# zhoujoey/ORB-SLAM3-Mac

Measured on AMD Instinct MI355X. Metric: ORB extract+match frames/sec, higher is better.
Workload: dtype u8; 1 GPU; vga: synthetic 640x480 batch=1024 per GPU, 8-level pyramid, 1000 feats/frame, ORB extract + Hamming 2-NN match (Frame.cc:1146) + SearchForInitialization (ORBmatcher.cc:710) vs successor frame; pipelines=1, matchers=side by side (two contexts), frames_total=1024

## Files before the change

orb-slam3-mac_amd/csrc/bf2nn_kernels.hip:

```cpp
#include "orb_internal.h"
#include "ctx_internal.h"
#include <climits>
#include <cstdlib>
#include <cstring>
#include <type_traits>

extern "C" int orbhip_descriptor_distance(const uint8_t *a32, const uint8_t *b32)
{
    int dist = 0;
    for (int i = 0; i < 8; i++) {
        uint32_t pa, pb;
        memcpy(&pa, a32 + 4 * i, 4); memcpy(&pb, b32 + 4 * i, 4);
        uint32_t v = pa ^ pb;
        v = v - ((v >> 1) & 0x55555555);
        v = (v & 0x33333333) + ((v >> 2) & 0x33333333);
        dist += (((v + (v >> 4)) & 0xF0F0F0F) * 0x1010101) >> 24;
    }
    return dist;
}

#define BF_TILE 256
__device__ __forceinline__ bool bf_slice(const int32_t *nA, const int32_t *nB, const int32_t *monoA, const int32_t *monoB, int pair, int max_n,
                                         int &na, int &nb, int &ma, int &mb)
{
    na = nA[pair]; nb = nB[pair]; ma = 0; mb = 0;
    if (!monoA) return true;
    if (na > max_n || nb > max_n) return false;
    ma = min(max(monoA[pair], 0), max(na, 0)); mb = min(max(monoB[pair], 0), max(nb, 0));
    na -= ma; nb -= mb;
    return true;
}
template <bool MONO>
__global__ __launch_bounds__(256) void k_bf2nn(const uint8_t *descA, const int32_t *nA, size_t strideA,
                                               const uint8_t *descB, const int32_t *nB, size_t strideB,
                                               int max_n, double ratio, int32_t *idx2, int32_t *dist2, uint8_t *accept,
                                               const int32_t *monoA, const int32_t *monoB)
{
    __shared__ uint4 tile[BF_TILE * 2];
    const int pair = blockIdx.y, tid = threadIdx.x;
    int na, nb, ma, mb;
    if (!bf_slice(nA, nB, MONO ? monoA : nullptr, monoB, pair, max_n, na, nb, ma, mb)) return;
    const int q = blockIdx.x * 256 + tid;
    if (blockIdx.x * 256 >= na) return;
    const uint4 *A = reinterpret_cast<const uint4 *>(descA + (size_t)pair * strideA) + 2 * (size_t)ma;
    const uint4 *B = reinterpret_cast<const uint4 *>(descB + (size_t)pair * strideB) + 2 * (size_t)mb;
    uint4 a0 = make_uint4(0, 0, 0, 0), a1 = a0;
    if (q < na) { a0 = A[2 * q]; a1 = A[2 * q + 1]; }
    uint32_t kb = 0xFFFFFFFFu, ks = 0xFFFFFFFFu;
    for (int t0 = 0; t0 < nb; t0 += BF_TILE) {
        const int tn = min(BF_TILE, nb - t0);
        __syncthreads();
        for (int i = tid; i < tn * 2; i += 256) tile[i] = B[2 * t0 + i];
        __syncthreads();
#pragma unroll 4
        for (int j = 0; j < tn; j++) {
            const uint32_t key = ((uint32_t)hamming256(a0, a1, tile[2 * j], tile[2 * j + 1]) << 16) | (uint32_t)(t0 + j);
            ks = min(ks, max(kb, key));
            kb = min(kb, key);
        }
    }
    if (q < na) {
        const int best = kb == 0xFFFFFFFFu ? INT_MAX : (int)(kb >> 16), second = ks == 0xFFFFFFFFu ? INT_MAX : (int)(ks >> 16);
        const int bi = kb == 0xFFFFFFFFu ? -1 : (int)(kb & 0xFFFFu), si = ks == 0xFFFFFFFFu ? -1 : (int)(ks & 0xFFFFu);
        const size_t o = ((size_t)pair * max_n + q) * 2;
        idx2[o] = bi; idx2[o + 1] = si; dist2[o] = best; dist2[o + 1] = second;
        accept[(size_t)pair * max_n + q] = (si >= 0 && (double)(float)best < (double)(float)second * ratio) ? 1 : 0;
    }
}

#define BFM_ROWB 272
typedef int bfm_v4i __attribute__((ext_vector_type(4)));
typedef int bfm_v16i __attribute__((ext_vector_type(16)));
__device__ __forceinline__ uint32_t bfm_widen4(uint32_t nib) { return __umul24(nib, 0x00204081u) & 0x01010101u; }
__device__ __forceinline__ uint32_t bfm_widen4_pm(uint32_t nib)
{
    const uint32_t s = bfm_widen4(nib);
    return ((s << 8) - s) | 0x01010101u;
}
#define BFM_WAVES 8
template <bool MONO>
__global__ __launch_bounds__(64 * BFM_WAVES, 4) void k_bf2nn_mfma(const uint8_t *descA, const int32_t *nA, size_t strideA,
                                                    const uint8_t *descB, const int32_t *nB, size_t strideB,
                                                    int max_n, double ratio, int32_t *idx2, int32_t *dist2, uint8_t *accept,
                                                    const int32_t *monoA, const int32_t *monoB)
{
    __shared__ __attribute__((aligned(16))) uint8_t Bx[2 * 64 * BFM_ROWB];
    static_assert(BFM_WAVES * 2 * 8 * 64 * 4 <= 2 * 64 * BFM_ROWB, "the merge area (half of the rows at a time) fits the tile buffers");
    const int pair = blockIdx.y, tid = threadIdx.x, lane = tid & 63, wave = tid >> 6;
    int na, nb, ma, mb;
    if (!bf_slice(nA, nB, MONO ? monoA : nullptr, monoB, pair, max_n, na, nb, ma, mb)) return;
    const int q0 = blockIdx.x * (32 * BFM_WAVES);
    if (q0 >= na) return;
    const uint32_t *A = reinterpret_cast<const uint32_t *>(descA + (size_t)pair * strideA) + 8 * (size_t)ma;
    const uint32_t *B = reinterpret_cast<const uint32_t *>(descB + (size_t)pair * strideB) + 8 * (size_t)mb;
    const int r = lane & 31, h = lane >> 5;
    const int qrow = q0 + 32 * wave + r;
    bfm_v4i af[8];
    int pa_row = 0;
    {
        uint32_t w[8];
#pragma unroll
        for (int m = 0; m < 8; m++) { w[m] = qrow < na ? A[(size_t)8 * qrow + m] : 0u; pa_row += __popc(w[m]); }
#pragma unroll
        for (int m = 0; m < 8; m++) {
            const uint32_t hw = (w[m] >> (16 * h)) & 0xFFFFu;
            af[m] = (bfm_v4i){(int)bfm_widen4_pm(hw & 15u), (int)bfm_widen4_pm((hw >> 4) & 15u), (int)bfm_widen4_pm((hw >> 8) & 15u), (int)bfm_widen4_pm(hw >> 12)};
        }
        asm volatile("" : "+v"(pa_row));
    }
    uint32_t k1[16], k2[16];
#pragma unroll
    for (int g = 0; g < 16; g++) { k1[g] = 0xFFFFFFFFu; k2[g] = 0xFFFFFFFFu; }
    const int sc = tid >> 3, sm = tid & 7;
    auto fetch = [&](int t0, uint32_t &w0) { w0 = (t0 + sc < nb) ? B[(uint32_t)(8 * (t0 + sc) + sm)] : 0u; };
    auto widen = [&](int bufi, uint32_t w) {
        uint4 lo = make_uint4(bfm_widen4(w & 15u), bfm_widen4((w >> 4) & 15u), bfm_widen4((w >> 8) & 15u), bfm_widen4((w >> 12) & 15u));
        uint4 hi = make_uint4(bfm_widen4((w >> 16) & 15u), bfm_widen4((w >> 20) & 15u), bfm_widen4((w >> 24) & 15u), bfm_widen4(w >> 28));
        uint4 *dst = reinterpret_cast<uint4 *>(&Bx[bufi * 64 * BFM_ROWB + sc * BFM_ROWB + sm * 32]);
        dst[0] = lo; dst[1] = hi;
    };
    uint32_t nw0;
    fetch(0, nw0);
    widen(0, nw0);
    __syncthreads();
    const bfm_v16i zero = {0, 0, 0, 0, 0, 0, 0, 0, 0, 0, 0, 0, 0, 0, 0, 0};
    bfm_v16i accA = zero, accB = zero;
    uint32_t baseB = 0;
    auto retire = [&](const bfm_v16i &acc, uint32_t base, int g) {
        const uint32_t key = ((uint32_t)acc[g] << 16) + base;
        asm("v_med3_u32 %1, %0, %2, %1\n\tv_min_u32 %0, %0, %2" : "+v"(k1[g]), "+v"(k2[g]) : "v"(key));
    };
    auto key_base = [&](int col) { return (col < nb ? (uint32_t)col : (0x40000000u | (uint32_t)col)) + (256u << 16); };
    const uint8_t *bx0 = &Bx[r * BFM_ROWB + h * 16];
    int buf = 0, t0 = 0;
    auto tile = [&](auto first) {
        constexpr bool FIRST = decltype(first)::value;
        const bool more = t0 + 64 < nb;
        if (more) fetch(t0 + 64, nw0);
        const uint8_t *bx = bx0 + buf * 64 * BFM_ROWB;
        auto rd = [&](int q) { return *reinterpret_cast<const bfm_v4i *>(bx + (q >> 3) * 32 * BFM_ROWB + (q & 7) * 32); };
        bfm_v4i bq[4];
#pragma unroll
        for (int q = 0; q < 4; q++) bq[q] = rd(q);
        if constexpr (!FIRST) {
#pragma unroll
            for (int g = 0; g < 4; g++) retire(accB, baseB, g);
        }
        const uint32_t baseA = key_base(t0 + r);
#pragma unroll
        for (int m = 0; m < 8; m++) {
            accA = __builtin_amdgcn_mfma_i32_32x32x32_i8(af[m], bq[m & 3], m ? accA : zero, 0, 0, 0);
            bq[m & 3] = rd(m + 4);
            if constexpr (!FIRST) {
                retire(accB, baseB, 4 + 3 * (m >> 1) + 2 * (m & 1));
                if (!(m & 1)) retire(accB, baseB, 5 + 3 * (m >> 1));
            }
            __builtin_amdgcn_sched_barrier(0);
        }
        baseB = key_base(t0 + 32 + r);
#pragma unroll
        for (int m = 0; m < 8; m++) {
            accB = __builtin_amdgcn_mfma_i32_32x32x32_i8(af[m], bq[m & 3], m ? accB : zero, 0, 0, 0);
            if (m < 4) bq[m & 3] = rd(m + 12);
            if (m) {
                const int g0 = (16 * (m - 1) + 6) / 7, g1 = (16 * m + 6) / 7;
#pragma unroll
                for (int g = g0; g < g1; g++) retire(accA, baseA, g);
            }
            __builtin_amdgcn_sched_barrier(0);
        }
        if (more) widen(buf ^ 1, nw0);
        __syncthreads();
        t0 += 64; buf ^= 1;
    };
    if (32 < nb) tile(std::true_type());
    while (t0 + 32 < nb) tile(std::false_type());
    if (t0 < nb) {
        const uint8_t *bx = bx0 + buf * 64 * BFM_ROWB;
        bfm_v4i bq[8];
#pragma unroll
        for (int m = 0; m < 8; m++) bq[m] = *reinterpret_cast<const bfm_v4i *>(bx + m * 32);
#pragma unroll
        for (int m = 0; m < 8; m++) accA = __builtin_amdgcn_mfma_i32_32x32x32_i8(af[m], bq[m], m ? accA : zero, 0, 0, 0);
        if (t0) {
#pragma unroll
            for (int g = 0; g < 16; g++) retire(accB, baseB, g);
        }
        const uint32_t baseA = key_base(t0 + r);
#pragma unroll
        for (int g = 0; g < 16; g++) retire(accA, baseA, g);
        __syncthreads();
    } else if (nb > 0) {
#pragma unroll
        for (int g = 0; g < 16; g++) retire(accB, baseB, g);
    }
    uint32_t (*kout)[2][8][64] = reinterpret_cast<uint32_t (*)[2][8][64]>(&Bx[0]);
#pragma unroll
    for (int part = 0; part < 2; part++) {
        if (part) __syncthreads();
#pragma unroll
        for (int g = 0; g < 8; g++) { kout[wave][0][g][lane] = k1[8 * part + g]; kout[wave][1][g][lane] = k2[8 * part + g]; }
        __syncthreads();
        const int row = 16 * part + (lane >> 2), g = (row & 3) + 4 * ((row >> 3) & 1), hh = (row >> 2) & 1;
        const int unbias = __shfl(pa_row, row, 64) - 256;
        uint32_t kb = 0xFFFFFFFFu, ks = 0xFFFFFFFFu;
#pragma unroll
        for (int c = 0; c < 8; c++) {
            const int cc = 32 * hh + 8 * (lane & 3) + ((c + (lane >> 2)) & 7);
            const uint32_t a1 = kout[wave][0][g][cc], a2 = kout[wave][1][g][cc];
            ks = min(min(ks, a2), max(kb, a1));
            kb = min(kb, a1);
        }
#pragma unroll
        for (int s = 1; s < 4; s <<= 1) {
            const uint32_t pb = __shfl_xor(kb, s, 64), ps = __shfl_xor(ks, s, 64);
            ks = min(min(ks, ps), max(kb, pb));
            kb = min(kb, pb);
        }
        const int q = q0 + 32 * wave + row;
        if ((lane & 3) == 0 && q < na) {
            const bool hb = !(kb & 0x40000000u), hs = !(ks & 0x40000000u);
            const int best = hb ? (int)(kb >> 16) + unbias : INT_MAX, second = hs ? (int)(ks >> 16) + unbias : INT_MAX;
            const int bi = hb ? (int)(kb & 0xFFFFu) : -1, si = hs ? (int)(ks & 0xFFFFu) : -1;
            const size_t o = ((size_t)pair * max_n + q) * 2;
            idx2[o] = bi; idx2[o + 1] = si; dist2[o] = best; dist2[o + 1] = second;
            accept[(size_t)pair * max_n + q] = (si >= 0 && (double)(float)best < (double)(float)second * ratio) ? 1 : 0;
        }
    }
}

extern "C" int orbhip_match_bf2nn_device(orbhip_ctx *ctx, const uint8_t *d_descA, const int32_t *d_nA, size_t strideA,
                                         const uint8_t *d_descB, const int32_t *d_nB, size_t strideB, int pairs,
                                         int max_n, double ratio, int32_t *d_idx2, int32_t *d_dist2, uint8_t *d_accept)
{
    if (!ctx || !d_descA || !d_descB || !d_nA || !d_nB || pairs <= 0 || max_n <= 0 || max_n > 65535 || !d_idx2 || !d_dist2 || !d_accept)
        return ORBHIP_E_BADARG;
    if (hipSetDevice(orbhip_ctx_device_internal(ctx)) != hipSuccess) return ORBHIP_E_HIP;
    if (max_n >= 64 && !getenv("ORBHIP_BF2NN_VALU")) {
        dim3 grid((max_n + 32 * BFM_WAVES - 1) / (32 * BFM_WAVES), pairs);
        hipLaunchKernelGGL(k_bf2nn_mfma<false>, grid, dim3(64 * BFM_WAVES), 0, orbhip_ctx_stream_internal(ctx), d_descA, d_nA, strideA, d_descB, d_nB,
                           strideB, max_n, ratio, d_idx2, d_dist2, d_accept, nullptr, nullptr);
    } else {
        dim3 grid((max_n + 255) / 256, pairs);
        hipLaunchKernelGGL(k_bf2nn<false>, grid, dim3(256), 0, orbhip_ctx_stream_internal(ctx), d_descA, d_nA, strideA, d_descB, d_nB,
                           strideB, max_n, ratio, d_idx2, d_dist2, d_accept, nullptr, nullptr);
    }
    return hipGetLastError() == hipSuccess ? ORBHIP_OK : ORBHIP_E_HIP;
}

int orbhip_bf2nn_slices_internal(orbhip_ctx *ctx, const uint8_t *d_descA, const int32_t *d_nA, const int32_t *d_monoA, size_t strideA,
                                 const uint8_t *d_descB, const int32_t *d_nB, const int32_t *d_monoB, size_t strideB, int pairs, int max_n,
                                 double ratio, int32_t *d_idx2, int32_t *d_dist2, uint8_t *d_accept)
{
    if (max_n >= 64 && !getenv("ORBHIP_BF2NN_VALU")) {
        dim3 grid((max_n + 32 * BFM_WAVES - 1) / (32 * BFM_WAVES), pairs);
        hipLaunchKernelGGL(k_bf2nn_mfma<true>, grid, dim3(64 * BFM_WAVES), 0, orbhip_ctx_stream_internal(ctx), d_descA, d_nA, strideA, d_descB, d_nB,
                           strideB, max_n, ratio, d_idx2, d_dist2, d_accept, d_monoA, d_monoB);
    } else {
        dim3 grid((max_n + 255) / 256, pairs);
        hipLaunchKernelGGL(k_bf2nn<true>, grid, dim3(256), 0, orbhip_ctx_stream_internal(ctx), d_descA, d_nA, strideA, d_descB, d_nB,
                           strideB, max_n, ratio, d_idx2, d_dist2, d_accept, d_monoA, d_monoB);
    }
    return hipGetLastError() == hipSuccess ? ORBHIP_OK : ORBHIP_E_HIP;
}
```

Measured before the change: 363,500 frames/s.

## Fold column index into MFMA accumulator to skip per-element key building

```diff
diff --git a/orb-slam3-mac_amd/csrc/bf2nn_kernels.hip b/orb-slam3-mac_amd/csrc/bf2nn_kernels.hip
--- a/orb-slam3-mac_amd/csrc/bf2nn_kernels.hip
+++ b/orb-slam3-mac_amd/csrc/bf2nn_kernels.hip
@@ -78,7 +78,15 @@
     return ((s << 8) - s) | 0x01010101u;
 }
 #define BFM_WAVES 8
-template <bool MONO>
+#define BFM_S 64
+#define BFM_NONE 0xFC000
+__device__ __forceinline__ uint32_t bfm_widen4_pmS(uint32_t nib)
+{
+    uint32_t s = bfm_widen4(nib);
+    asm("" : "+v"(s));
+    return (s << 7) | 0x40404040u;
+}
+template <bool MONO, bool TIDX>
 __global__ __launch_bounds__(64 * BFM_WAVES, 4) void k_bf2nn_mfma(const uint8_t *descA, const int32_t *nA, size_t strideA,
                                                     const uint8_t *descB, const int32_t *nB, size_t strideB,
                                                     int max_n, double ratio, int32_t *idx2, int32_t *dist2, uint8_t *accept,
@@ -91,6 +99,7 @@
     if (!bf_slice(nA, nB, MONO ? monoA : nullptr, monoB, pair, max_n, na, nb, ma, mb)) return;
     const int q0 = blockIdx.x * (32 * BFM_WAVES);
     if (q0 >= na) return;
+    if (TIDX && nb > 32 * BFM_S) return;
     const uint32_t *A = reinterpret_cast<const uint32_t *>(descA + (size_t)pair * strideA) + 8 * (size_t)ma;
     const uint32_t *B = reinterpret_cast<const uint32_t *>(descB + (size_t)pair * strideB) + 8 * (size_t)mb;
     const int r = lane & 31, h = lane >> 5;
@@ -104,13 +113,14 @@
 #pragma unroll
         for (int m = 0; m < 8; m++) {
             const uint32_t hw = (w[m] >> (16 * h)) & 0xFFFFu;
-            af[m] = (bfm_v4i){(int)bfm_widen4_pm(hw & 15u), (int)bfm_widen4_pm((hw >> 4) & 15u), (int)bfm_widen4_pm((hw >> 8) & 15u), (int)bfm_widen4_pm(hw >> 12)};
+            if constexpr (TIDX) af[m] = (bfm_v4i){(int)bfm_widen4_pmS(hw & 15u), (int)bfm_widen4_pmS((hw >> 4) & 15u), (int)bfm_widen4_pmS((hw >> 8) & 15u), (int)bfm_widen4_pmS(hw >> 12)};
+            else af[m] = (bfm_v4i){(int)bfm_widen4_pm(hw & 15u), (int)bfm_widen4_pm((hw >> 4) & 15u), (int)bfm_widen4_pm((hw >> 8) & 15u), (int)bfm_widen4_pm(hw >> 12)};
         }
         asm volatile("" : "+v"(pa_row));
     }
     uint32_t k1[16], k2[16];
 #pragma unroll
-    for (int g = 0; g < 16; g++) { k1[g] = 0xFFFFFFFFu; k2[g] = 0xFFFFFFFFu; }
+    for (int g = 0; g < 16; g++) { k1[g] = TIDX ? (uint32_t)BFM_NONE : 0xFFFFFFFFu; k2[g] = k1[g]; }
     const int sc = tid >> 3, sm = tid & 7;
     auto fetch = [&](int t0, uint32_t &w0) { w0 = (t0 + sc < nb) ? B[(uint32_t)(8 * (t0 + sc) + sm)] : 0u; };
     auto widen = [&](int bufi, uint32_t w) {
@@ -127,21 +137,49 @@
     bfm_v16i accA = zero, accB = zero;
     uint32_t baseB = 0;
     auto retire = [&](const bfm_v16i &acc, uint32_t base, int g) {
-        const uint32_t key = ((uint32_t)acc[g] << 16) + base;
-        asm("v_med3_u32 %1, %0, %2, %1\n\tv_min_u32 %0, %0, %2" : "+v"(k1[g]), "+v"(k2[g]) : "v"(key));
+        if constexpr (TIDX) {
+            if (g == 0) {
+                const int x = acc[0], b1 = (int)k1[0], b2 = (int)k2[0];
+                k2[0] = (uint32_t)max(min(b2, x), min(max(b2, x), b1));
+                k1[0] = (uint32_t)min(b1, x);
+                asm volatile("" : "+v"(k1[0]), "+v"(k2[0]));
+            } else {
+                asm volatile("v_med3_i32 %1, %0, %2, %1\n\tv_min_i32 %0, %0, %2" : "+v"(k1[g]), "+v"(k2[g]) : "v"(acc[g]));
+            }
+        } else {
+            const uint32_t key = ((uint32_t)acc[g] << 16) + base;
+            asm("v_med3_u32 %1, %0, %2, %1\n\tv_min_u32 %0, %0, %2" : "+v"(k1[g]), "+v"(k2[g]) : "v"(key));
+        }
     };
+    auto retire_last = [&](const bfm_v16i &acc, int col0, uint32_t base) {
+        if constexpr (TIDX) {
+            const bool real = col0 + r < nb;
+#pragma unroll
+            for (int g = 0; g < 16; g++) {
+                const int x = real ? acc[g] : BFM_NONE;
+                asm volatile("v_med3_i32 %1, %0, %2, %1\n\tv_min_i32 %0, %0, %2" : "+v"(k1[g]), "+v"(k2[g]) : "v"(x));
+            }
+        } else {
+#pragma unroll
+            for (int g = 0; g < 16; g++) retire(acc, base, g);
+        }
+    };
+    const long a9 = h ? 0 : 1;
+    auto open_chain = [&](int col0) { return __builtin_amdgcn_mfma_i32_32x32x16_i8(a9, (long)(col0 >> 5), zero, 0, 0, 0); };
     auto key_base = [&](int col) { return (col < nb ? (uint32_t)col : (0x40000000u | (uint32_t)col)) + (256u << 16); };
     const uint8_t *bx0 = &Bx[r * BFM_ROWB + h * 16];
     int buf = 0, t0 = 0;
+    constexpr int RING = TIDX ? 2 : 4;
     auto tile = [&](auto first) {
         constexpr bool FIRST = decltype(first)::value;
         const bool more = t0 + 64 < nb;
         if (more) fetch(t0 + 64, nw0);
         const uint8_t *bx = bx0 + buf * 64 * BFM_ROWB;
         auto rd = [&](int q) { return *reinterpret_cast<const bfm_v4i *>(bx + (q >> 3) * 32 * BFM_ROWB + (q & 7) * 32); };
-        bfm_v4i bq[4];
-#pragma unroll
-        for (int q = 0; q < 4; q++) bq[q] = rd(q);
+        bfm_v4i bq[RING];
+#pragma unroll
+        for (int q = 0; q < RING; q++) bq[q] = rd(q);
+        if constexpr (TIDX) { accA = open_chain(t0); __builtin_amdgcn_sched_barrier(0); }
         if constexpr (!FIRST) {
 #pragma unroll
             for (int g = 0; g < 4; g++) retire(accB, baseB, g);
@@ -149,8 +187,8 @@
         const uint32_t baseA = key_base(t0 + r);
 #pragma unroll
         for (int m = 0; m < 8; m++) {
-            accA = __builtin_amdgcn_mfma_i32_32x32x32_i8(af[m], bq[m & 3], m ? accA : zero, 0, 0, 0);
-            bq[m & 3] = rd(m + 4);
+            accA = __builtin_amdgcn_mfma_i32_32x32x32_i8(af[m], bq[m % RING], (TIDX || m) ? accA : zero, 0, 0, 0);
+            bq[m % RING] = rd(m + RING);
             if constexpr (!FIRST) {
                 retire(accB, baseB, 4 + 3 * (m >> 1) + 2 * (m & 1));
                 if (!(m & 1)) retire(accB, baseB, 5 + 3 * (m >> 1));
@@ -158,10 +196,11 @@
             __builtin_amdgcn_sched_barrier(0);
         }
         baseB = key_base(t0 + 32 + r);
+        if constexpr (TIDX) { accB = open_chain(t0 + 32); __builtin_amdgcn_sched_barrier(0); }
 #pragma unroll
         for (int m = 0; m < 8; m++) {
-            accB = __builtin_amdgcn_mfma_i32_32x32x32_i8(af[m], bq[m & 3], m ? accB : zero, 0, 0, 0);
-            if (m < 4) bq[m & 3] = rd(m + 12);
+            accB = __builtin_amdgcn_mfma_i32_32x32x32_i8(af[m], bq[(8 + m) % RING], (TIDX || m) ? accB : zero, 0, 0, 0);
+            if (8 + m + RING < 16) bq[(8 + m) % RING] = rd(8 + m + RING);
             if (m) {
                 const int g0 = (16 * (m - 1) + 6) / 7, g1 = (16 * m + 6) / 7;
 #pragma unroll
@@ -180,19 +219,24 @@
         bfm_v4i bq[8];
 #pragma unroll
         for (int m = 0; m < 8; m++) bq[m] = *reinterpret_cast<const bfm_v4i *>(bx + m * 32);
-#pragma unroll
-        for (int m = 0; m < 8; m++) accA = __builtin_amdgcn_mfma_i32_32x32x32_i8(af[m], bq[m], m ? accA : zero, 0, 0, 0);
+        if constexpr (TIDX) accA = open_chain(t0);
+#pragma unroll
+        for (int m = 0; m < 8; m++) accA = __builtin_amdgcn_mfma_i32_32x32x32_i8(af[m], bq[m], (TIDX || m) ? accA : zero, 0, 0, 0);
         if (t0) {
 #pragma unroll
             for (int g = 0; g < 16; g++) retire(accB, baseB, g);
         }
-        const uint32_t baseA = key_base(t0 + r);
-#pragma unroll
-        for (int g = 0; g < 16; g++) retire(accA, baseA, g);
+        retire_last(accA, t0, key_base(t0 + r));
         __syncthreads();
     } else if (nb > 0) {
-#pragma unroll
-        for (int g = 0; g < 16; g++) retire(accB, baseB, g);
+        retire_last(accB, t0 - 32, baseB);
+    }
+    if constexpr (TIDX) {
+        static_assert(BFM_S == 64 && BFM_NONE == ((1 << 14) - 256) * BFM_S, "to_key: 16 - log2(S) = 10, and (BFM_NONE / S + 256) << 16 is bit 30");
+        const uint32_t kc = (256u << 16) + (uint32_t)r;
+        auto to_key = [&](uint32_t x) { return (x << 10) + kc - (x & (BFM_S - 1)) * 992u; };
+#pragma unroll
+        for (int g = 0; g < 16; g++) { k1[g] = to_key(k1[g]); k2[g] = to_key(k2[g]); }
     }
     uint32_t (*kout)[2][8][64] = reinterpret_cast<uint32_t (*)[2][8][64]>(&Bx[0]);
 #pragma unroll
@@ -238,7 +282,8 @@
     if (hipSetDevice(orbhip_ctx_device_internal(ctx)) != hipSuccess) return ORBHIP_E_HIP;
     if (max_n >= 64 && !getenv("ORBHIP_BF2NN_VALU")) {
         dim3 grid((max_n + 32 * BFM_WAVES - 1) / (32 * BFM_WAVES), pairs);
-        hipLaunchKernelGGL(k_bf2nn_mfma<false>, grid, dim3(64 * BFM_WAVES), 0, orbhip_ctx_stream_internal(ctx), d_descA, d_nA, strideA, d_descB, d_nB,
+        auto kern = max_n <= 32 * BFM_S ? k_bf2nn_mfma<false, true> : k_bf2nn_mfma<false, false>;
+        hipLaunchKernelGGL(kern, grid, dim3(64 * BFM_WAVES), 0, orbhip_ctx_stream_internal(ctx), d_descA, d_nA, strideA, d_descB, d_nB,
                            strideB, max_n, ratio, d_idx2, d_dist2, d_accept, nullptr, nullptr);
     } else {
         dim3 grid((max_n + 255) / 256, pairs);
@@ -254,7 +299,8 @@
 {
     if (max_n >= 64 && !getenv("ORBHIP_BF2NN_VALU")) {
         dim3 grid((max_n + 32 * BFM_WAVES - 1) / (32 * BFM_WAVES), pairs);
-        hipLaunchKernelGGL(k_bf2nn_mfma<true>, grid, dim3(64 * BFM_WAVES), 0, orbhip_ctx_stream_internal(ctx), d_descA, d_nA, strideA, d_descB, d_nB,
+        auto kern = max_n <= 32 * BFM_S ? k_bf2nn_mfma<true, true> : k_bf2nn_mfma<true, false>;
+        hipLaunchKernelGGL(kern, grid, dim3(64 * BFM_WAVES), 0, orbhip_ctx_stream_internal(ctx), d_descA, d_nA, strideA, d_descB, d_nB,
                            strideB, max_n, ratio, d_idx2, d_dist2, d_accept, d_monoA, d_monoB);
     } else {
         dim3 grid((max_n + 255) / 256, pairs);
```

Measured after the change: 365,100 frames/s (median of 4 runs). About the same (+0.4%).
